# lucidrains/voicebox-pytorch

Measured on AMD Instinct MI355X. Metric: mel-frames/sec train-step (fwd+bwd+allreduce+clip+Adam), higher is better.
Workload: dtype f16/bf16 (fp16 forward operands, bf16 backward operands, fp32 accumulate/master); 1 GPU; VoiceBox dim 512 depth 12 heads 16 unconditional, 8x1024 frames per GPU, train; global_batch=8, seq_len=1024, parallelism=dp1

## Files before the change

### include/vbx.h

```cpp
#ifndef VBX_H
#define VBX_H
#include <stddef.h>
#include <stdint.h>

#ifdef __cplusplus
extern "C" {
#endif

#define VBX_VERSION 1

enum { VBX_OK = 0, VBX_EINVAL = -1, VBX_EUNSUPPORTED = -2, VBX_EWORKSPACE = -3 };

int vbx_version(void);
const char* vbx_last_error(void);
int vbx_check_device(int dev);

enum { VBX_GEMM_NT = 0, VBX_GEMM_NN = 1, VBX_GEMM_TN = 2 };

enum {
  VBX_EPI_BF16 = 0,
  VBX_EPI_F32 = 1,
  VBX_EPI_QKV = 2,
  VBX_EPI_GEGLU = 3,
  VBX_EPI_SPLITK = 4,
// ... 426 lines not shown

size_t vbx_model_wpack_bytes(const vbx_model* m);
size_t vbx_model_act_bytes(const vbx_model* m);
int vbx_model_pack_weights(const vbx_model* m, void* stream);
int vbx_model_adaln_factors(const vbx_model* m, const float** dada, const float** temb, long* w_off, void** dst_f16);
long vbx_model_sq_partials(const vbx_model* m, long* ranges );
int vbx_model_adam_segments(const vbx_model* m, long n_flat, vbx_adam_seg* out, int max_segs, long* total_blocks);
int vbx_model_forward(const vbx_model* m, const vbx_io* io, void* stream);
int vbx_model_adaln_table(const vbx_model* m, const float* temb, int n, float* ada, void* stream);
int vbx_model_backward_head(const vbx_model* m, const vbx_io* io, const float* gscale, void* stream);
int vbx_model_backward_layer(const vbx_model* m, const vbx_io* io, int layer, void* stream);
int vbx_model_backward_embed(const vbx_model* m, const vbx_io* io, void* stream);
int vbx_wgrad_overlap(int on);
int vbx_wgrad_overlap_forks(void);
int vbx_wgrad_overlap_delay(float side_us, float main_us);

void* vbx_model_debug_ptr(const vbx_model* m, const char* name, int layer);

int vbx_split3_f16(const float* src, long rows, int K, long ld, void* dst_f16, int Kp, void* stream);
int vbx_pack_weight3(const float* src, int src_rows, int src_cols, void* dst_f16, int dst_rows, int dst_cols, int rowmap, int F,
                     void* stream);
int vbx_qknorm_rope_f32(const float* raw, int B, int H, int Np, float qk_scale, const float* q_gamma, const float* k_gamma,
                        const float* rot_cos, const float* rot_sin, float* q32, float* k32, float* v32, void* q16, void* k16,
                        void* qb, void* kb, void* v_bf16, void* v16, float* q_rnorm, float* k_rnorm,
                        float q16_scale ,
                        void* stream);
int vbx_attn_fwd_f32(const float* q, const float* k, const float* v, const uint8_t* mask, float* out32, void* out16, void* out_bf16,
                     float* lse, int B, int H, int Np, float scale, void* stream);
int vbx_attn_fwd_f32_dropout(const float* q, const float* k, const float* v, const uint8_t* mask, float* out32, void* out16,
                             void* out_bf16, float* lse, int B, int H, int Np, float scale, const void* bits_rm, float p, void* stream);
// ... 22 lines not shown
```

### voicebox-pytorch_amd/csrc/runtime.hip

```cpp
#include "common.hpp"
#include "wgrad_overlap_plan.hpp"
#include <stdlib.h>
#include <algorithm>
#include <string.h>
#include <string>
#include <vector>

namespace {

inline size_t al256(size_t x) { return (x + 255) & ~(size_t)255; }

struct Carver {
  char* base;
  size_t off = 0;
  explicit Carver(void* b) : base((char*)b) {}
  template <class T>
  T* take(size_t n) {
    off = al256(off);
    T* p = base ? (T*)(base + off) : nullptr;
    off += n * sizeof(T);
    return p;
  }
};

// ... 295 lines not shown
  }
  ~ProfScope() {
    if (idx >= 0) (void)hipEventRecord(g_prof.recs[idx].e1, st);
  }
};

#define CK(x)                 \
  do {                        \
    int rc__ = (x);           \
    if (rc__ != 0) return rc__; \
  } while (0)

struct WgoSide {
  hipStream_t st = nullptr;
  hipEvent_t ev[wgrad_overlap::EV_N] = {};
};
int g_wgo_on = -1;
float g_wgo_delay[2] = {0.f, 0.f};
int g_wgo_forks = 0;
bool wgo_enabled() {
  if (g_wgo_on < 0) {
    const char* e = getenv("VBX_WGRAD_OVERLAP");
    g_wgo_on = e ? (atoi(e) != 0) : 1;
  }
  return g_wgo_on != 0;
}
WgoSide* wgo_side(bool create) {
  static WgoSide* sides[64] = {};
  int dev = 0;
  if (hipGetDevice(&dev) != hipSuccess || dev < 0 || dev >= 64) return nullptr;
  if (sides[dev] || !create) return sides[dev];
  WgoSide* s = new WgoSide;
  int least = 0, greatest = 0;
  bool ok = hipDeviceGetStreamPriorityRange(&least, &greatest) == hipSuccess &&
            hipStreamCreateWithPriority(&s->st, hipStreamNonBlocking, least) == hipSuccess;
  for (int i = 0; ok && i < wgrad_overlap::EV_N; i++) ok = hipEventCreateWithFlags(&s->ev[i], hipEventDisableTiming) == hipSuccess;
  if (!ok) {
    for (auto e : s->ev) if (e) (void)hipEventDestroy(e);
    if (s->st) (void)hipStreamDestroy(s->st);
    delete s;
    (void)hipGetLastError();
    return nullptr;
  }
  return sides[dev] = s;
}
bool capturing(hipStream_t st) {
  hipStreamCaptureStatus cs = hipStreamCaptureStatusNone;
  return hipStreamIsCapturing(st, &cs) != hipSuccess || cs != hipStreamCaptureStatusNone;
}
int wgo_sync(WgoSide* sd, hipStream_t main_st, wgrad_overlap::Point p, int l, int L) {
  if (!sd) return 0;
  const wgrad_overlap::Sync s = wgrad_overlap::sync_at(p, l, L);
  if (s.kind == wgrad_overlap::SYNC_NONE) return 0;
  hipStream_t st = s.stream == wgrad_overlap::MAIN ? main_st : sd->st;
  const hipError_t e = s.kind == wgrad_overlap::SYNC_RECORD ? hipEventRecord(sd->ev[s.ev], st) : hipStreamWaitEvent(st, sd->ev[s.ev], 0);
  VBX_REQUIRE(e == hipSuccess, "weight-gradient overlap: event %s failed (%s)", s.kind == wgrad_overlap::SYNC_RECORD ? "record" : "wait",
              hipGetErrorString(e));
  return 0;
}
struct WgoGuard {
  WgoSide* sd = nullptr;
  bool forked = false, ok = false;
  int done(int rc) { ok = rc == 0; return rc; }
  ~WgoGuard() {
    if (forked && !ok && sd) (void)hipStreamSynchronize(sd->st);
  }
};
bool defers(const vbx_model* m) { return m->defer_reduce && !m->gateloop && !m->unet && (m->plain_norm || m->adaln_factors); }
struct { const void* act = nullptr; int dxb = 0, dqkv = 0; } g_last_copy;

int check_model(const vbx_model* m) {
  VBX_REQUIRE(m && m->params && m->off && m->wpack && m->act && m->rot_cos && m->rot_sin, "vbx_model: null field");
  VBX_REQUIRE(m->D % 64 == 0 && m->D <= 2048, "vbx_model: dim must be a multiple of 64 and <= 2048 (got %d)", m->D);
  VBX_REQUIRE(m->H > 0 && m->H % 2 == 0, "vbx_model: heads must be even (dim_head is fixed at 64)");
  VBX_REQUIRE(m->Th % 8 == 0 && m->L > 0 && m->B > 0 && m->N > 0 && m->R >= 0 && m->F > 0, "vbx_model: bad dims");
  VBX_REQUIRE(m->ksize >= 1 && m->ksize <= 31 && (m->ksize & 1), "vbx_model: conv_pos_embed_kernel_size must be odd and <= 31 (got %d)", m->ksize);
  VBX_REQUIRE(m->E >= 0 && m->E % 8 == 0 && (m->E == 0 || (m->V1 > 0 && !m->stack_only)), "vbx_model: bad dim_cond_emb / table size");
  const long DT = (long)m->D * m->Th;
  for (int l = 0; l < m->L; l++) {
    const long* o = m->off + VBX_NG + (long)l * VBX_NL;
    if (m->plain_norm) continue;
    VBX_REQUIRE(o[VBX_L_B1W] == o[VBX_L_G1W] + DT && o[VBX_L_G2W] == o[VBX_L_B1W] + DT && o[VBX_L_B2W] == o[VBX_L_G2W] + DT,
                "vbx_model: adaLN weights of layer %d are not contiguous in (g1,b1,g2,b2) order", l);
// ... 146 lines not shown
  const float* P = m->params;
  const long* G = m->off;
  const bool tr = m->training != 0;

  if (m->precise) {
    std::vector<VbxPreciseLayer> pl(d.L);
    for (int l = 0; l < d.L; l++) {
      const ALayer& y = a.layer[l];
      pl[l] = VbxPreciseLayer{y.hn1, y.q16, y.k16, y.qb, y.kb, y.v, y.vh, y.oh, y.o, y.hn2, y.gh, y.g, tr ? y.h1 : nullptr,
                              y.qrn, y.krn, y.lse, w.layer[l].b1, y.hg, y.glp, y.gls, tr ? y.glh : nullptr, (unsigned*)y.dbr, (unsigned*)y.dbc};
    }
    VbxPreciseActs pa{a.four, a.pre, a.temb, a.ada, a.e, a.pred, a.per_b, a.xs.data(), pl.data(), a.embed_in, a.embed_inh, a.hf};
    return vbx_forward_precise(m, io, &pa, stream);
  }

  if (m->stack_only) {
    CK(vbx_stack_input(io->x, d.R ? P + G[VBX_P_REG] : nullptr, a.xs[0], d.B, d.N, d.R, d.D, stream));
    if (!m->plain_norm) CK(vbx_adaln_proj_fwd(io->cond, w.adah, w.bada, a.ada, d.B, d.Th, d.J, 4 * d.D, stream));
  } else {
  if (io->ada_table) {
    VBX_REQUIRE(!tr && io->ada_counter && io->ada_stride >= 1,
                "vbx_model_forward: ada_table is an inference-only input and needs ada_counter and ada_stride >= 1");
    CK(vbx_ada_select(a.ada, d.L, d.B, 4 * d.D, io->ada_table, io->ada_counter, io->ada_stride, io->ada_slot, stream));
  } else {
  CK(vbx_time_embed_fwd(io->times, P + G[VBX_P_SINW], P + G[VBX_P_T1W], P + G[VBX_P_T1B], a.four, a.pre, a.temb, d.B, d.D,
                        d.Th, stream));
  CK(vbx_adaln_proj_fwd(a.temb, w.adah, w.bada, a.ada, d.B, d.Th, d.J, 4 * d.D, stream));
  }
  if (d.Lc) {
    CK(vbx_proj_in_embed(io->x, io->cond, w.pinh, P + G[VBX_P_PINB], io->cond_mask, io->drop_mask, io->null_cond, a.embed_inh,
                         a.embed_in, a.xcb, d.B, d.N, d.Lc, d.D, d.E, stream));
    if (d.E) {
      VBX_REQUIRE(io->cond_ids && io->T > 0, "vbx_model_forward: a text-conditioned model needs cond_ids");
      CK(vbx_embed_text_cols(io->drop_mask, io->cond_ids, io->T, P + G[VBX_P_CEMB], d.E, io->null_id, a.embed_inh, a.embed_in, d.B,
                             d.N, d.D, d.Ke, stream));
    }
  } else if (d.E) {
    VBX_REQUIRE(io->cond_ids && io->T > 0, "vbx_model_forward: a text-conditioned model needs cond_ids");
    CK(vbx_pack_embed_input_text(io->x, io->cond, io->cond_mask, io->drop_mask, io->null_cond, io->cond_ids, io->T,
                                 P + G[VBX_P_CEMB], d.E, io->null_id, a.embed_inh, a.embed_in, d.B, d.N, d.Din, stream));
  } else {
    CK(vbx_pack_embed_input(io->x, io->cond, io->cond_mask, a.embed_inh, a.embed_in, d.B, d.N, d.Din, stream));
  }
  CK(gemm_nt(a.embed_inh, d.Ke, w.embh, d.Ke, (int)d.M0, d.D, d.Ke, VBX_EPI_F32, a.e, d.D, P + G[VBX_P_EMBB], nullptr,
             nullptr, nullptr, st));
  if (m->packed)
    CK(vbx_convpos_fwd_segs(a.e, P + G[VBX_P_CONVW], P + G[VBX_P_CONVB], d.R ? P + G[VBX_P_REG] : nullptr, io->seg_start, io->seg_klen,
                            io->tile_seg, a.xs[0], d.N, d.R, d.D, d.ks, stream));
  else
  CK(vbx_convpos_fwd(a.e, P + G[VBX_P_CONVW], P + G[VBX_P_CONVB], io->attn_mask, d.R ? P + G[VBX_P_REG] : nullptr, a.xs[0],
                     d.B, d.N, d.R, d.D, d.ks, stream));
  }

  for (int l = 0; l < d.L; l++) {
    const long* o = m->off + VBX_NG + (long)l * VBX_NL;
    const ALayer& y = a.layer[l];
    const float* ada_l = a.ada + (size_t)l * d.B * 4 * d.D;
    const int S = m->gateloop ? 3 : 2;
    float* x0 = layer_input(m, a, l);
    float* x_in = m->gateloop ? a.xs[S * l + 1] : x0;
    float* x_mid = a.xs[S * l + S - 1];
    float* x_out = a.xs[S * l + S];
    if (m->unet && l >= d.L / 2) {
      CK(vbx_unet_cat(a.xs[S * l], a.xs[S * (d.L - 1 - l)], m->skip_scale, a.cat16, nullptr, d.M, d.D, stream));
      CK(gemm_nt(a.cat16, 2 * d.D, w.layer[l].skwh, 2 * d.D, (int)d.M, d.D, 2 * d.D, VBX_EPI_F32, x0, d.D, P + o[VBX_L_SKB], nullptr,
                 nullptr, nullptr, st));
    }
    if (m->gateloop) {
// ... 39 lines not shown
    if (drop_on && m->ff_dropout > 0.f)
      CK(vbx_dropout_rows(y.gh, tr ? y.g : nullptr, d.M, d.Fp, d.Fp, io->drop_seed, 2u * l + 1u, m->ff_dropout, stream));
    { ProfScope ps("fwd ff_out", st);
      CK(gemm_nt(y.gh, d.Fp, w.layer[l].w2h, d.Fp, (int)d.M, d.D, d.Fp, VBX_EPI_F32, x_out, d.D, P + o[VBX_L_FF2B], x_mid, nullptr,
                 nullptr, st)); }
  }
  if (m->stack_only)
    return vbx_rmsnorm_fwd_f32(a.xs[(m->gateloop ? 3 : 2) * d.L], P + G[VBX_P_FNG], nullptr, 0, io->pred, d.B, d.Np, d.R, d.N, d.D,
                               stream);
  CK(vbx_rmsnorm_fwd(a.xs[(m->gateloop ? 3 : 2) * d.L], P + G[VBX_P_FNG], nullptr, 0, a.hf, a.hfh, d.B, d.Np, m->packed ? 0 : d.R, d.N, d.D,
                     stream));
  if (d.Dop != d.Do) {
    CK(gemm_nt(a.hfh, d.D, w.predh, d.D, (int)d.M0, d.Dop, d.D, VBX_EPI_F32, a.pred, d.Dop, nullptr, nullptr, nullptr, nullptr, st));
    if (io->pred) CK(vbx_copy_cols_f32(a.pred, d.Dop, io->pred, d.M0, d.Do, stream));
    if (io->target) CK(vbx_masked_mse_fwd_ld(a.pred, d.Dop, io->target, io->loss_mask, a.per_b, io->loss, d.B, d.N, d.Do, stream));
    return 0;
  }
  float* pred = io->pred ? io->pred : a.pred;
  CK(gemm_nt(a.hfh, d.D, w.predh, d.D, (int)d.M0, d.Do, d.D, VBX_EPI_F32, pred, d.Do, nullptr, nullptr, nullptr, nullptr, st));
  if (io->target) CK(vbx_masked_mse_fwd(pred, io->target, io->loss_mask, a.per_b, io->loss, d.B, d.N, d.Do, stream));
  return 0;
}

extern "C" int vbx_model_backward_head(const vbx_model* m, const vbx_io* io, const float* gscale, void* stream) {
  CK(check_model(m));
  VBX_REQUIRE(m->training && m->grads && io && io->target && (m->stack_only || io->loss_mask),
              "vbx_model_backward_head: needs a training forward");
  hipStream_t st = (hipStream_t)stream;
  const Dims d = dims_of(m);
  WPack w;
  carve_wpack(m, w);
  Acts a;
  carve_acts(m, a);
  const float* P = m->params;
  float* Gd = m->grads;
  const long* G = m->off;
  WgoGuard guard;
  guard.sd = capturing(st) ? nullptr : wgo_side(false);
  guard.forked = guard.sd != nullptr;
  CK(wgo_sync(guard.sd, st, wgrad_overlap::PT_HEAD_BEGIN, -1, d.L));
  u16* const dxb = defers(m) ? a.copy[wgrad_overlap::BUF_DXB][wgrad_overlap::dxb_read_copy(d.L - 1)] : a.dxb;
  g_last_copy.act = m->act; g_last_copy.dxb = (int)(dxb != a.dxb ? wgrad_overlap::dxb_read_copy(d.L - 1) : 0);
  if (m->stack_only) {
    CK(vbx_pack_weight(io->target, (int)d.M0, d.D, a.dhn, nullptr, (int)d.M0, d.D, 0, 0, stream));
  } else {
    const float* pred = io->pred ? io->pred : a.pred;
    if (d.Dop != d.Do)
      CK(vbx_masked_mse_bwd_ld(a.pred, d.Dop, io->target, io->loss_mask, a.per_b, gscale, a.dpb, d.B, d.N, d.Do, stream));
    else
      CK(vbx_masked_mse_bwd(pred, io->target, io->loss_mask, a.per_b, gscale, nullptr, a.dpb, d.B, d.N, d.Do, stream));
    CK(wgrad(a.dpb, d.Dop, a.hf, d.D, d.Dop, d.D, d.M0, a.slabs, Gd + G[VBX_P_PREDW], d.Do, d.D, 0, 0, st));
    CK(gemm_nn_bf16(a.dpb, d.Dop, w.pred, d.D, (int)d.M0, d.D, d.Dop, a.dhn, d.D, st));
  }
  if (hipMemsetAsync(a.dx, 0, (size_t)d.M * d.D * sizeof(float), st) != hipSuccess ||
      hipMemsetAsync(dxb, 0, (size_t)d.M * d.D * sizeof(u16), st) != hipSuccess) {
    vbx_set_error("vbx_model_backward_head: memset failed");
    return VBX_EINVAL;
  }
  CK(vbx_rmsnorm_bwd(a.xs[(m->gateloop ? 3 : 2) * d.L], P + G[VBX_P_FNG], 0, a.dhn, nullptr, a.dx, dxb, a.npart, nullptr, d.B, d.Np, d.R, d.N, d.D,
                     stream));
  CK(vbx_reduce_norm_partials(a.npart, a.tmp2d, 0, d.B, vbx_rmsnorm_bwd_chunks(d.N), d.D, 1, stream));
  CK(vbx_sum_rows_f32(a.tmp2d, 1, d.D, Gd + G[VBX_P_FNG], d.D, 0, stream));
  return guard.done(0);
}

struct SqLayout { long off[4], per_layer; };
static SqLayout sq_layout(const Dims& d) {
  SqLayout q;
  const long n[4] = {vbx_splitk_reduce_blocks(d.D, d.Fp), vbx_splitk_reduce_blocks(2 * d.Fp, d.D), vbx_splitk_reduce_blocks(d.D, d.I),
                     vbx_splitk_reduce_blocks(3 * d.I, d.D)};
  q.off[0] = 0;
  for (int i = 1; i < 4; i++) q.off[i] = q.off[i - 1] + n[i - 1];
  q.per_layer = q.off[3] + n[3];
  return q;
}
extern "C" long vbx_model_sq_partials(const vbx_model* m, long* ranges) {
  if (check_model(m) != 0) return 0;
// ... 139 lines not shown
  namespace wgo = wgrad_overlap;
  auto copy_of = [&](wgo::Buf b) { return pl.defer ? a.copy[b][wgo::write_copy(b, l)] : a.copy[b][0]; };
  u16* const dxb_in = pl.defer ? a.copy[wgo::BUF_DXB][wgo::dxb_read_copy(l)] : a.dxb;
  u16* const dxb_out = copy_of(wgo::BUF_DXB);
  u16* const dh1 = copy_of(wgo::BUF_DH1);
  u16* const dqkv = copy_of(wgo::BUF_DQKV);
  u16* dxb_attn = wgp ? copy_of(wgo::BUF_DXB2) : dxb_in;
  g_last_copy.act = m->act; g_last_copy.dxb = pl.defer ? wgo::write_copy(wgo::BUF_DXB, l) : 0; g_last_copy.dqkv = pl.defer ? wgo::write_copy(wgo::BUF_DQKV, l) : 0;
  const bool cap = capturing(st);
  const bool fork = pl.defer && wgp && wgo_enabled() && !g_prof.on && !cap;
  WgoGuard guard;
  guard.sd = cap ? nullptr : wgo_side(fork);
  VBX_REQUIRE(!fork || guard.sd, "vbx_model_backward_layer: could not create the weight-gradient side stream");
  if (fork && g_wgo_delay[1] > 0.f) CK(vbx_stream_delay(g_wgo_delay[1], stream));
  CK(wgo_sync(guard.sd, st, wgo::PT_LAYER_BEGIN, l, d.L));
  float* const slabs = fork ? a.slabs_side : a.slabs;
  const size_t sfl = a.slab_floats;
  const SqLayout sql = sq_layout(d);
  float* const sqb = m->sq_partials ? m->sq_partials + (long)l * sql.per_layer : nullptr;
  auto sq_at = [&](int i) { return sqb ? sqb + sql.off[i] : nullptr; };

  { ProfScope ps("dgrad ff_out", st); CK(gemm_nn_bf16(dxb_in, d.D, wl.w2, d.Fp, M, d.Fp, d.D, a.dg, d.Fp, st)); }
  CK(wgrad(dxb_in, d.D, y.g, d.Fp, d.D, d.Fp, d.M, slabs, Gd + o[VBX_L_FF2W], d.D, d.F, 0, 0, st, &wj, wgp, gs, sq_at(0)));
  if (drop_on && m->ff_dropout > 0.f)
    CK(vbx_dropout_rows(nullptr, a.dg, d.M, d.Fp, d.Fp, io->drop_seed, 2u * l + 1u, m->ff_dropout, stream));
  CK(vbx_geglu_bwd_colsum(y.h1, a.dg, dh1, M, d.Fp, csl, stream));
  { ProfScope ps("dgrad ff_in", st); CK(gemm_nn_bf16(dh1, 2 * d.Fp, wl.w1, d.D, M, d.D, 2 * d.Fp, a.dhn, d.D, st)); }
  CK(wgrad(dh1, 2 * d.Fp, y.hn2, d.D, 2 * d.Fp, d.D, d.M, slabs + sfl, Gd + o[VBX_L_FF1W], 2 * d.F, d.D, 1, d.F, st, &wj, wgp, gs, sq_at(1)));
  CK(vbx_rmsnorm_bwd(x_mid, g2, gstride, a.dhn, a.dx, a.dx, dxb_attn, npart, cpart, d.B, d.Np, 0, d.Np, d.D, stream));

// ... 20 lines not shown
    if (g_wgo_delay[0] > 0.f) CK(vbx_stream_delay(g_wgo_delay[0], side));
    if (wgg.n) CK(vbx_gemm_tn_splitk_grouped(wgg.d, wgg.n, side));
    CK(wgo_sync(guard.sd, st, wgo::PT_SIDE_GEMM_DONE, l, d.L));
    if (wj.n) CK(vbx_splitk_reduce_multi(&wj, side));
    CK(wgo_sync(guard.sd, st, wgo::PT_SIDE_REDUCE_DONE, l, d.L));
  } else {
    if (wgg.n) { ProfScope ps("wgrad (4 GEMMs)", st); CK(vbx_gemm_tn_splitk_grouped(wgg.d, wgg.n, stream)); }
    if (wj.n) { ProfScope ps("wgrad slab reduce", st); CK(vbx_splitk_reduce_multi(&wj, stream)); }
  }
  CK(vbx_rmsnorm_bwd(x_in, g1, gstride, a.dhn, a.dx, a.dx, dxb_out, npart2, nullptr, d.B, d.Np, 0, d.Np, d.D, stream));

  vbx_mr_jobs jb{};
  if (!pl.defer) {
    layer_reduce_jobs(m, d, a, pl, l, 0, jb);
    CK(vbx_multi_reduce(&jb, stream));
  } else if (l == 0) {
    ProfScope ps("partials reduce (all)", st);
    for (int ll = d.L - 1; ll >= 0; ll--) {
      layer_reduce_jobs(m, d, a, pl, ll, ll, jb);
      if (jb.n + 8 > VBX_MR_MAX || ll == 0) {
        CK(vbx_multi_reduce(&jb, stream));
        jb.n = 0;
      }
    }
  }

  if (m->gateloop) CK(backward_gateloop(m, d, w, a, l, stream));
  if (m->unet) CK(backward_unet(m, d, w, a, l, stream));
  if (m->plain_norm) return guard.done(0);
  if (pl.ada_all) {
    if (l == 0) {
      ProfScope ps("adaLN dtemb (all)", st);
      CK(vbx_adaln_dtemb_all(w.adah, a.dada, a.dtemb, a.ada_scratch, d.L, d.B, d.Th, 4 * d.D, stream));
    }
    return guard.done(0);
  }
  return guard.done(vbx_adaln_proj_bwd(m->stack_only ? io->cond : a.temb, w.adah + (size_t)l * 4 * d.D * d.Th, dada_l,
                            m->adaln_factors ? nullptr : Gd + o[VBX_L_G1W], Gd + o[VBX_L_G1B], a.dtemb,
                            a.ada_scratch, d.B, d.Th, 4 * d.D, l == d.L - 1 ? 0 : 1, stream));
}

extern "C" int vbx_model_backward_embed(const vbx_model* m, const vbx_io* io, void* stream) {
  CK(check_model(m));
  VBX_REQUIRE(m->training && m->grads && io && (m->stack_only ? io->dx != nullptr : io->times != nullptr),
              "vbx_model_backward_embed: needs a training forward");
  hipStream_t st = (hipStream_t)stream;
  const Dims d = dims_of(m);
  WPack w;
  carve_wpack(m, w);
  Acts a;
  carve_acts(m, a);
  const float* P = m->params;
  float* Gd = m->grads;
  const long* G = m->off;
  WgoGuard guard;
  guard.sd = capturing(st) ? nullptr : wgo_side(false);
  guard.forked = guard.sd != nullptr;
  if (m->stack_only) {
    CK(vbx_stack_input_bwd(a.dx, io->dx, d.R ? Gd + G[VBX_P_REG] : nullptr, d.B, d.N, d.R, d.D, stream));
    if (!m->plain_norm && io->dcond &&
        hipMemcpyAsync(io->dcond, a.dtemb, (size_t)d.B * d.Th * sizeof(float), hipMemcpyDeviceToDevice, st) != hipSuccess) {
      vbx_set_error("vbx_model_backward_embed: copy of d(cond) failed");
      return VBX_EINVAL;
    }
    return guard.done(wgo_sync(guard.sd, st, wgrad_overlap::PT_EMBED_END, -1, d.L));
  }
  CK(vbx_convpos_bwd(a.e, P + G[VBX_P_CONVW], P + G[VBX_P_CONVB], io->attn_mask, a.dx, a.dpre, a.de, a.deb, a.wpart,
                     d.R ? Gd + G[VBX_P_REG] : nullptr, d.B, d.N, d.R, d.D, d.ks, stream));
  CK(vbx_conv_wgrad_finalize(a.wpart, vbx_convpos_bwd_chunks(d.B, d.N), d.D, d.ks, Gd + G[VBX_P_CONVW], Gd + G[VBX_P_CONVB], stream));
  CK(wgrad(a.deb, d.D, a.embed_in, d.Ke, d.D, d.Ke, d.M0, a.slabs, Gd + G[VBX_P_EMBW], d.D, d.Ke, 0, 0, st));
  if (d.E) {
    WPack w;
    carve_wpack(m, w);
    CK(gemm_nn_bf16(a.deb, d.D, w.embb + d.Din, d.Ke, (int)d.M0, d.E, d.D, a.demb, d.E, st));
    if (hipMemsetAsync(Gd + G[VBX_P_CEMB], 0, (size_t)m->V1 * d.E * sizeof(float), st) != hipSuccess) {
      vbx_set_error("vbx_model_backward_embed: memset of the embedding gradient failed");
      return VBX_EINVAL;
    }
    CK(vbx_cond_emb_bwd(a.demb, d.E, io->cond_ids, io->T, io->drop_mask, io->null_id, Gd + G[VBX_P_CEMB], d.B, d.N, d.E, stream));
  }
  if (d.Lc) {
    WPack w;
    carve_wpack(m, w);
    CK(gemm_nn_bf16(a.deb, d.D, w.embb, d.Ke, (int)d.M0, d.D, d.D, a.dxc, d.D, st));
    CK(gemm_nn_bf16(a.deb, d.D, w.embb + d.D + d.E, d.Ke, (int)d.M0, d.D, d.D, a.dxc + (size_t)d.M0 * d.D, d.D, st));
    vbx_gemm_desc g{};
    g.mode = VBX_GEMM_TN; g.epilogue = VBX_EPI_SPLITK; g.M = d.D; g.N = d.Kp; g.K = (int)(2 * d.M0); g.lda = d.D; g.ldb = d.Kp;
    g.A = a.dxc; g.B = a.xcb; g.C = a.slabs; g.splits = wgrad_splits(d.D, d.Kp, 2 * d.M0);
    CK(vbx_gemm(&g, st));
    CK(vbx_proj_in_wgrad_reduce(a.slabs, g.splits, d.D, d.Lc, Gd + G[VBX_P_PINW], Gd + G[VBX_P_PINB], stream));
  }
  CK(vbx_colsum_f32(a.de, (int)d.M0, d.D, d.D, Gd + G[VBX_P_EMBB], a.cs_scratch, stream));
  CK(vbx_time_embed_bwd(io->times, P + G[VBX_P_SINW], P + G[VBX_P_T1W], a.four, a.pre, a.dtemb, Gd + G[VBX_P_SINW],
                        Gd + G[VBX_P_T1W], Gd + G[VBX_P_T1B], a.tscratch, d.B, d.D, d.Th, stream));
  return guard.done(wgo_sync(guard.sd, st, wgrad_overlap::PT_EMBED_END, -1, d.L));
}

extern "C" int vbx_model_adam_segments(const vbx_model* m, long n_flat, vbx_adam_seg* out, int max_segs, long* total_blocks) {
  CK(check_model(m));
  VBX_REQUIRE(n_flat > 0 && total_blocks, "vbx_model_adam_segments: bad args");
  const Dims d = dims_of(m);
  WPack w;
  carve_wpack(m, w);
  const long* G = m->off;
  std::vector<vbx_adam_seg> ps;
  auto add = [&](long off, long rows, long cols, void* b, void* h16, float* f32, int ld, int rowmap, int F) {
    vbx_adam_seg s{};
    s.off = off; s.count = rows * cols; s.dst_bf16 = b; s.dst_f16 = h16; s.dst_f32 = f32; s.cols = (int)cols; s.dst_ld = ld;
    s.rowmap = rowmap; s.F = F;
    ps.push_back(s);
// ... 55 lines not shown
}

extern "C" int vbx_wgrad_overlap(int on) {
  VBX_REQUIRE(on == 0 || on == 1, "vbx_wgrad_overlap: 0 in line, 1 on the side stream");
  g_wgo_on = on;
  return 0;
}
extern "C" int vbx_wgrad_overlap_forks(void) { return g_wgo_forks; }
extern "C" int vbx_wgrad_overlap_delay(float side_us, float main_us) {
  VBX_REQUIRE(side_us >= 0.f && side_us <= 2000.f && main_us >= 0.f && main_us <= 2000.f, "vbx_wgrad_overlap_delay: 0 .. 2000 us each");
  g_wgo_delay[0] = side_us;
  g_wgo_delay[1] = main_us;
  return 0;
}

extern "C" int vbx_prof_enable(int on) {
  for (auto& r : g_prof.recs) { (void)hipEventDestroy(r.e0); (void)hipEventDestroy(r.e1); }
  g_prof.recs.clear();
  g_prof.on = on != 0;
  return 0;
}
extern "C" int vbx_prof_collect(vbx_prof_entry* out, int max_entries) {
  VBX_REQUIRE(out && max_entries > 0, "vbx_prof_collect: bad args");
  g_prof.on = false;
  int n = 0;
  for (auto& r : g_prof.recs) {
    float ms = 0.f;
    if (hipEventSynchronize(r.e1) != hipSuccess || hipEventElapsedTime(&ms, r.e0, r.e1) != hipSuccess) continue;
    int k = 0;
    for (; k < n; k++)
// ... 39 lines not shown
```

Measured before the change: 1.005 million mel-frames/s.

## Move small independent step branches onto an auxiliary stream with event joins

Adds a second low-priority auxiliary stream and an event plan that moves small independent launches off the main stream. In backward these are the to_pred weight gradient, the final-norm gradient reduce, the grouped per-layer partial multi-reduces, the adaLN dtemb pass and the time-embedding backward. The forward head region is defined, but the plan's region_kept excludes it, so the time-embed and adaLN projection still run inline. The goal is to hide these latency-bound kernels behind main-stream GEMM work, at the cost of more event records and waits plus added cross-stream hazard complexity.

```diff
diff --git a/include/vbx.h b/include/vbx.h
--- a/include/vbx.h
+++ b/include/vbx.h
@@ -464,6 +464,9 @@
 int vbx_wgrad_overlap(int on);
 int vbx_wgrad_overlap_forks(void);
 int vbx_wgrad_overlap_delay(float side_us, float main_us);
+int vbx_step_branches(int on);
+int vbx_step_branches_forks(void);
+int vbx_step_branches_delay(float aux_us, float main_us);
 
 void* vbx_model_debug_ptr(const vbx_model* m, const char* name, int layer);
 
diff --git a/voicebox-pytorch_amd/csrc/runtime.hip b/voicebox-pytorch_amd/csrc/runtime.hip
--- a/voicebox-pytorch_amd/csrc/runtime.hip
+++ b/voicebox-pytorch_amd/csrc/runtime.hip
@@ -1,5 +1,6 @@
 #include "common.hpp"
 #include "wgrad_overlap_plan.hpp"
+#include "step_branches_plan.hpp"
 #include <stdlib.h>
 #include <algorithm>
 #include <string.h>
@@ -333,10 +334,15 @@
 struct WgoSide {
   hipStream_t st = nullptr;
   hipEvent_t ev[wgrad_overlap::EV_N] = {};
+  hipStream_t aux = nullptr;
+  hipEvent_t evb[step_branches::EV_N] = {};
 };
 int g_wgo_on = -1;
 float g_wgo_delay[2] = {0.f, 0.f};
 int g_wgo_forks = 0;
+int g_sb_on = 1;
+float g_sb_delay[2] = {0.f, 0.f};
+int g_sb_forks = 0;
 bool wgo_enabled() {
   if (g_wgo_on < 0) {
     const char* e = getenv("VBX_WGRAD_OVERLAP");
@@ -352,11 +358,15 @@
   WgoSide* s = new WgoSide;
   int least = 0, greatest = 0;
   bool ok = hipDeviceGetStreamPriorityRange(&least, &greatest) == hipSuccess &&
-            hipStreamCreateWithPriority(&s->st, hipStreamNonBlocking, least) == hipSuccess;
+            hipStreamCreateWithPriority(&s->st, hipStreamNonBlocking, least) == hipSuccess &&
+            hipStreamCreateWithPriority(&s->aux, hipStreamNonBlocking, least) == hipSuccess;
   for (int i = 0; ok && i < wgrad_overlap::EV_N; i++) ok = hipEventCreateWithFlags(&s->ev[i], hipEventDisableTiming) == hipSuccess;
+  for (int i = 0; ok && i < step_branches::EV_N; i++) ok = hipEventCreateWithFlags(&s->evb[i], hipEventDisableTiming) == hipSuccess;
   if (!ok) {
     for (auto e : s->ev) if (e) (void)hipEventDestroy(e);
+    for (auto e : s->evb) if (e) (void)hipEventDestroy(e);
     if (s->st) (void)hipStreamDestroy(s->st);
+    if (s->aux) (void)hipStreamDestroy(s->aux);
     delete s;
     (void)hipGetLastError();
     return nullptr;
@@ -377,15 +387,40 @@
               hipGetErrorString(e));
   return 0;
 }
+int sb_sync(WgoSide* sd, hipStream_t main_st, step_branches::Point p, int l, int L, int per_layer, bool on) {
+  if (!sd) return 0;
+  const step_branches::Sync s = step_branches::sync_at(p, l, L, per_layer, on);
+  if (s.kind == step_branches::SYNC_NONE) return 0;
+  hipStream_t st = s.stream == step_branches::MAIN ? main_st : sd->aux;
+  const hipError_t e = s.kind == step_branches::SYNC_RECORD ? hipEventRecord(sd->evb[s.ev], st) : hipStreamWaitEvent(st, sd->evb[s.ev], 0);
+  VBX_REQUIRE(e == hipSuccess, "step branches: event %s failed (%s)", s.kind == step_branches::SYNC_RECORD ? "record" : "wait",
+              hipGetErrorString(e));
+  return 0;
+}
 struct WgoGuard {
   WgoSide* sd = nullptr;
   bool forked = false, ok = false;
   int done(int rc) { ok = rc == 0; return rc; }
   ~WgoGuard() {
-    if (forked && !ok && sd) (void)hipStreamSynchronize(sd->st);
+    if (forked && !ok && sd) {
+      (void)hipStreamSynchronize(sd->st);
+      (void)hipStreamSynchronize(sd->aux);
+    }
   }
 };
 bool defers(const vbx_model* m) { return m->defer_reduce && !m->gateloop && !m->unet && (m->plain_norm || m->adaln_factors); }
+bool sb_backward(const vbx_model* m, bool cap) {
+  return g_sb_on && defers(m) && group_wgrad() && wgo_enabled() && !g_prof.on && !cap && !m->stack_only && !m->precise;
+}
+int sb_fork(WgoGuard& guard, hipStream_t main_st, step_branches::Point fork, step_branches::Point begin, int l, int L, int per_layer) {
+  CK(sb_sync(guard.sd, main_st, fork, l, L, per_layer, true));
+  guard.forked = true;
+  g_sb_forks++;
+  if (g_sb_delay[1] > 0.f) CK(vbx_stream_delay(g_sb_delay[1], main_st));
+  CK(sb_sync(guard.sd, main_st, begin, l, L, per_layer, true));
+  if (g_sb_delay[0] > 0.f) CK(vbx_stream_delay(g_sb_delay[0], guard.sd->aux));
+  return 0;
+}
 struct { const void* act = nullptr; int dxb = 0, dqkv = 0; } g_last_copy;
 
 int check_model(const vbx_model* m) {
@@ -562,6 +597,15 @@
     return vbx_forward_precise(m, io, &pa, stream);
   }
 
+  namespace sb = step_branches;
+  WgoGuard guard;
+  const bool branch = tr && sb::region_on(sb::REG_FWD_HEAD, g_sb_on != 0) && !m->stack_only && !m->gateloop && !m->unet && !io->ada_table &&
+                      group_wgrad() && wgo_enabled() && !g_prof.on && !capturing(st);
+  if (branch) {
+    guard.sd = wgo_side(true);
+    VBX_REQUIRE(guard.sd, "vbx_model_forward: could not create the side streams");
+  }
+
   if (m->stack_only) {
     CK(vbx_stack_input(io->x, d.R ? P + G[VBX_P_REG] : nullptr, a.xs[0], d.B, d.N, d.R, d.D, stream));
     if (!m->plain_norm) CK(vbx_adaln_proj_fwd(io->cond, w.adah, w.bada, a.ada, d.B, d.Th, d.J, 4 * d.D, stream));
@@ -571,9 +615,12 @@
                 "vbx_model_forward: ada_table is an inference-only input and needs ada_counter and ada_stride >= 1");
     CK(vbx_ada_select(a.ada, d.L, d.B, 4 * d.D, io->ada_table, io->ada_counter, io->ada_stride, io->ada_slot, stream));
   } else {
+  if (branch) CK(sb_fork(guard, st, sb::PT_FWD_BEGIN, sb::PT_FWD_AUX_BEGIN, -1, d.L, 0));
+  void* const ts = branch ? (void*)guard.sd->aux : stream;
   CK(vbx_time_embed_fwd(io->times, P + G[VBX_P_SINW], P + G[VBX_P_T1W], P + G[VBX_P_T1B], a.four, a.pre, a.temb, d.B, d.D,
-                        d.Th, stream));
-  CK(vbx_adaln_proj_fwd(a.temb, w.adah, w.bada, a.ada, d.B, d.Th, d.J, 4 * d.D, stream));
+                        d.Th, ts));
+  CK(vbx_adaln_proj_fwd(a.temb, w.adah, w.bada, a.ada, d.B, d.Th, d.J, 4 * d.D, ts));
+  CK(sb_sync(guard.sd, st, sb::PT_FWD_AUX_END, -1, d.L, 0, branch));
   }
   if (d.Lc) {
     CK(vbx_proj_in_embed(io->x, io->cond, w.pinh, P + G[VBX_P_PINB], io->cond_mask, io->drop_mask, io->null_cond, a.embed_inh,
@@ -600,6 +647,7 @@
                      d.B, d.N, d.R, d.D, d.ks, stream));
   }
 
+  CK(sb_sync(guard.sd, st, sb::PT_FWD_LAYER0, -1, d.L, 0, branch));
   for (int l = 0; l < d.L; l++) {
     const long* o = m->off + VBX_NG + (long)l * VBX_NL;
     const ALayer& y = a.layer[l];
@@ -669,12 +717,12 @@
     CK(gemm_nt(a.hfh, d.D, w.predh, d.D, (int)d.M0, d.Dop, d.D, VBX_EPI_F32, a.pred, d.Dop, nullptr, nullptr, nullptr, nullptr, st));
     if (io->pred) CK(vbx_copy_cols_f32(a.pred, d.Dop, io->pred, d.M0, d.Do, stream));
     if (io->target) CK(vbx_masked_mse_fwd_ld(a.pred, d.Dop, io->target, io->loss_mask, a.per_b, io->loss, d.B, d.N, d.Do, stream));
-    return 0;
+    return guard.done(0);
   }
   float* pred = io->pred ? io->pred : a.pred;
   CK(gemm_nt(a.hfh, d.D, w.predh, d.D, (int)d.M0, d.Do, d.D, VBX_EPI_F32, pred, d.Do, nullptr, nullptr, nullptr, nullptr, st));
   if (io->target) CK(vbx_masked_mse_fwd(pred, io->target, io->loss_mask, a.per_b, io->loss, d.B, d.N, d.Do, stream));
-  return 0;
+  return guard.done(0);
 }
 
 extern "C" int vbx_model_backward_head(const vbx_model* m, const vbx_io* io, const float* gscale, void* stream) {
@@ -690,10 +738,15 @@
   const float* P = m->params;
   float* Gd = m->grads;
   const long* G = m->off;
+  namespace sb = step_branches;
+  const bool cap = capturing(st);
+  const bool branch = sb::region_on(sb::REG_BWD_HEAD, sb_backward(m, cap));
   WgoGuard guard;
-  guard.sd = capturing(st) ? nullptr : wgo_side(false);
+  guard.sd = cap ? nullptr : wgo_side(branch);
+  VBX_REQUIRE(!branch || guard.sd, "vbx_model_backward_head: could not create the side streams");
   guard.forked = guard.sd != nullptr;
   CK(wgo_sync(guard.sd, st, wgrad_overlap::PT_HEAD_BEGIN, -1, d.L));
+  CK(sb_sync(guard.sd, st, sb::PT_HEAD_BEGIN, -1, d.L, 0, branch));
   u16* const dxb = defers(m) ? a.copy[wgrad_overlap::BUF_DXB][wgrad_overlap::dxb_read_copy(d.L - 1)] : a.dxb;
   g_last_copy.act = m->act; g_last_copy.dxb = (int)(dxb != a.dxb ? wgrad_overlap::dxb_read_copy(d.L - 1) : 0);
   if (m->stack_only) {
@@ -704,7 +757,7 @@
       CK(vbx_masked_mse_bwd_ld(a.pred, d.Dop, io->target, io->loss_mask, a.per_b, gscale, a.dpb, d.B, d.N, d.Do, stream));
     else
       CK(vbx_masked_mse_bwd(pred, io->target, io->loss_mask, a.per_b, gscale, nullptr, a.dpb, d.B, d.N, d.Do, stream));
-    CK(wgrad(a.dpb, d.Dop, a.hf, d.D, d.Dop, d.D, d.M0, a.slabs, Gd + G[VBX_P_PREDW], d.Do, d.D, 0, 0, st));
+    if (!branch) CK(wgrad(a.dpb, d.Dop, a.hf, d.D, d.Dop, d.D, d.M0, a.slabs, Gd + G[VBX_P_PREDW], d.Do, d.D, 0, 0, st));
     CK(gemm_nn_bf16(a.dpb, d.Dop, w.pred, d.D, (int)d.M0, d.D, d.Dop, a.dhn, d.D, st));
   }
   if (hipMemsetAsync(a.dx, 0, (size_t)d.M * d.D * sizeof(float), st) != hipSuccess ||
@@ -714,8 +767,16 @@
   }
   CK(vbx_rmsnorm_bwd(a.xs[(m->gateloop ? 3 : 2) * d.L], P + G[VBX_P_FNG], 0, a.dhn, nullptr, a.dx, dxb, a.npart, nullptr, d.B, d.Np, d.R, d.N, d.D,
                      stream));
-  CK(vbx_reduce_norm_partials(a.npart, a.tmp2d, 0, d.B, vbx_rmsnorm_bwd_chunks(d.N), d.D, 1, stream));
-  CK(vbx_sum_rows_f32(a.tmp2d, 1, d.D, Gd + G[VBX_P_FNG], d.D, 0, stream));
+  hipStream_t hs = st;
+  if (branch) {
+    CK(sb_fork(guard, st, sb::PT_HEAD_FORK, sb::PT_HEAD_AUX_BEGIN, -1, d.L, 0));
+    hs = guard.sd->aux;
+    CK(wgrad(a.dpb, d.Dop, a.hf, d.D, d.Dop, d.D, d.M0, a.slabs, Gd + G[VBX_P_PREDW], d.Do, d.D, 0, 0, hs));
+  }
+  CK(vbx_reduce_norm_partials(a.npart, a.tmp2d, 0, d.B, vbx_rmsnorm_bwd_chunks(d.N), d.D, 1, hs));
+  CK(vbx_sum_rows_f32(a.tmp2d, 1, d.D, Gd + G[VBX_P_FNG], d.D, 0, hs));
+  CK(sb_sync(guard.sd, st, sb::PT_HEAD_AUX_DONE, -1, d.L, 0, branch));
+  CK(sb_sync(guard.sd, st, sb::PT_HEAD_AUX_JOIN, -1, d.L, 0, branch));
   return guard.done(0);
 }
 
@@ -885,6 +946,9 @@
   VBX_REQUIRE(!fork || guard.sd, "vbx_model_backward_layer: could not create the weight-gradient side stream");
   if (fork && g_wgo_delay[1] > 0.f) CK(vbx_stream_delay(g_wgo_delay[1], stream));
   CK(wgo_sync(guard.sd, st, wgo::PT_LAYER_BEGIN, l, d.L));
+  namespace sb = step_branches;
+  const bool tail = fork && sb::region_on(sb::REG_BWD_TAIL, sb_backward(m, cap));
+  CK(sb_sync(guard.sd, st, sb::PT_LAYER_BEGIN, l, d.L, 0, tail));
   float* const slabs = fork ? a.slabs_side : a.slabs;
   const size_t sfl = a.slab_floats;
   const SqLayout sql = sq_layout(d);
@@ -935,6 +999,20 @@
   if (!pl.defer) {
     layer_reduce_jobs(m, d, a, pl, l, 0, jb);
     CK(vbx_multi_reduce(&jb, stream));
+  } else if (tail) {
+    layer_reduce_jobs(m, d, a, pl, l, l, jb);
+    const int per_layer = jb.n;
+    jb.n = 0;
+    const int first = sb::mr_group_first(l, d.L, per_layer);
+    if (first >= 0) {
+      static_assert(sb::kMrMax == VBX_MR_MAX, "step_branches_plan.hpp restates VBX_MR_MAX");
+      VBX_REQUIRE((first - l + 1) * per_layer <= VBX_MR_MAX, "vbx_model_backward_layer: the reduce plan overfills a launch");
+      CK(sb_fork(guard, st, sb::PT_MR_FORK, sb::PT_MR_AUX_BEGIN, l, d.L, per_layer));
+      for (int ll = first; ll >= l; ll--) layer_reduce_jobs(m, d, a, pl, ll, ll, jb);
+      CK(vbx_multi_reduce(&jb, guard.sd->aux));
+      if (l == 0 && pl.ada_all) CK(vbx_adaln_dtemb_all(w.adah, a.dada, a.dtemb, a.ada_scratch, d.L, d.B, d.Th, 4 * d.D, guard.sd->aux));
+      CK(sb_sync(guard.sd, st, sb::PT_MR_AUX_END, l, d.L, per_layer, true));
+    }
   } else if (l == 0) {
     ProfScope ps("partials reduce (all)", st);
     for (int ll = d.L - 1; ll >= 0; ll--) {
@@ -950,7 +1028,7 @@
   if (m->unet) CK(backward_unet(m, d, w, a, l, stream));
   if (m->plain_norm) return guard.done(0);
   if (pl.ada_all) {
-    if (l == 0) {
+    if (l == 0 && !tail) {
       ProfScope ps("adaLN dtemb (all)", st);
       CK(vbx_adaln_dtemb_all(w.adah, a.dada, a.dtemb, a.ada_scratch, d.L, d.B, d.Th, 4 * d.D, stream));
     }
@@ -974,9 +1052,16 @@
   const float* P = m->params;
   float* Gd = m->grads;
   const long* G = m->off;
+  namespace sb = step_branches;
+  const bool cap = capturing(st);
   WgoGuard guard;
-  guard.sd = capturing(st) ? nullptr : wgo_side(false);
+  guard.sd = cap ? nullptr : wgo_side(false);
   guard.forked = guard.sd != nullptr;
+  const bool tail = guard.sd && sb::region_on(sb::REG_BWD_TAIL, sb_backward(m, cap));
+  auto join = [&]() -> int {
+    CK(wgo_sync(guard.sd, st, wgrad_overlap::PT_EMBED_END, -1, d.L));
+    return sb_sync(guard.sd, st, sb::PT_EMBED_END, -1, d.L, 0, tail);
+  };
   if (m->stack_only) {
     CK(vbx_stack_input_bwd(a.dx, io->dx, d.R ? Gd + G[VBX_P_REG] : nullptr, d.B, d.N, d.R, d.D, stream));
     if (!m->plain_norm && io->dcond &&
@@ -984,7 +1069,18 @@
       vbx_set_error("vbx_model_backward_embed: copy of d(cond) failed");
       return VBX_EINVAL;
     }
-    return guard.done(wgo_sync(guard.sd, st, wgrad_overlap::PT_EMBED_END, -1, d.L));
+    return guard.done(join());
+  }
+  auto time_bwd = [&](void* s) {
+    return vbx_time_embed_bwd(io->times, P + G[VBX_P_SINW], P + G[VBX_P_T1W], a.four, a.pre, a.dtemb, Gd + G[VBX_P_SINW],
+                              Gd + G[VBX_P_T1W], Gd + G[VBX_P_T1B], a.tscratch, d.B, d.D, d.Th, s);
+  };
+  if (tail) {
+    g_sb_forks++;
+    if (g_sb_delay[0] > 0.f) CK(vbx_stream_delay(g_sb_delay[0], guard.sd->aux));
+    CK(time_bwd(guard.sd->aux));
+    CK(sb_sync(guard.sd, st, sb::PT_EMBED_AUX_END, -1, d.L, 0, true));
+    if (g_sb_delay[1] > 0.f) CK(vbx_stream_delay(g_sb_delay[1], stream));
   }
   CK(vbx_convpos_bwd(a.e, P + G[VBX_P_CONVW], P + G[VBX_P_CONVB], io->attn_mask, a.dx, a.dpre, a.de, a.deb, a.wpart,
                      d.R ? Gd + G[VBX_P_REG] : nullptr, d.B, d.N, d.R, d.D, d.ks, stream));
@@ -1012,9 +1108,8 @@
     CK(vbx_proj_in_wgrad_reduce(a.slabs, g.splits, d.D, d.Lc, Gd + G[VBX_P_PINW], Gd + G[VBX_P_PINB], stream));
   }
   CK(vbx_colsum_f32(a.de, (int)d.M0, d.D, d.D, Gd + G[VBX_P_EMBB], a.cs_scratch, stream));
-  CK(vbx_time_embed_bwd(io->times, P + G[VBX_P_SINW], P + G[VBX_P_T1W], a.four, a.pre, a.dtemb, Gd + G[VBX_P_SINW],
-                        Gd + G[VBX_P_T1W], Gd + G[VBX_P_T1B], a.tscratch, d.B, d.D, d.Th, stream));
-  return guard.done(wgo_sync(guard.sd, st, wgrad_overlap::PT_EMBED_END, -1, d.L));
+  if (!tail) CK(time_bwd(stream));
+  return guard.done(join());
 }
 
 extern "C" int vbx_model_adam_segments(const vbx_model* m, long n_flat, vbx_adam_seg* out, int max_segs, long* total_blocks) {
@@ -1100,6 +1195,19 @@
   return 0;
 }
 
+extern "C" int vbx_step_branches(int on) {
+  VBX_REQUIRE(on == 0 || on == 1, "vbx_step_branches: 0 in line, 1 on the AUX stream");
+  g_sb_on = on;
+  return 0;
+}
+extern "C" int vbx_step_branches_forks(void) { return g_sb_forks; }
+extern "C" int vbx_step_branches_delay(float aux_us, float main_us) {
+  VBX_REQUIRE(aux_us >= 0.f && aux_us <= 2000.f && main_us >= 0.f && main_us <= 2000.f, "vbx_step_branches_delay: 0 .. 2000 us each");
+  g_sb_delay[0] = aux_us;
+  g_sb_delay[1] = main_us;
+  return 0;
+}
+
 extern "C" int vbx_prof_enable(int on) {
   for (auto& r : g_prof.recs) { (void)hipEventDestroy(r.e0); (void)hipEventDestroy(r.e1); }
   g_prof.recs.clear();
diff --git a/voicebox-pytorch_amd/csrc/step_branches_plan.hpp b/voicebox-pytorch_amd/csrc/step_branches_plan.hpp
--- /dev/null
+++ b/voicebox-pytorch_amd/csrc/step_branches_plan.hpp
@@ -0,0 +1,282 @@
+#pragma once
+#include <string.h>
+
+#include "wgrad_overlap_plan.hpp"
+
+namespace step_branches {
+namespace wgo = wgrad_overlap;
+
+enum Stream { MAIN = wgo::MAIN, SIDE = wgo::SIDE, AUX, STREAM_N };
+
+enum Region { REG_FWD_HEAD, REG_BWD_HEAD, REG_BWD_TAIL, REG_N };
+constexpr bool region_kept(Region r) { return r != REG_FWD_HEAD; }
+
+enum Launch { LA_TIME_EMBED_FWD, LA_ADALN_PROJ_FWD, LA_TO_PRED_WGRAD, LA_FNORM_REDUCE, LA_MULTI_REDUCE, LA_ADALN_DTEMB, LA_TIME_EMBED_BWD };
+constexpr Region region_of(Launch la) {
+  return la <= LA_ADALN_PROJ_FWD ? REG_FWD_HEAD : (la <= LA_FNORM_REDUCE ? REG_BWD_HEAD : REG_BWD_TAIL);
+}
+constexpr bool region_on(Region r, bool on) { return on && region_kept(r); }
+constexpr Stream stream_of(Launch la, bool on) { return region_on(region_of(la), on) ? AUX : MAIN; }
+
+constexpr int kMrMax = 48, kMrRoom = 8;
+constexpr int mr_group_first(int l, int L, int per_layer) {
+  int n = 0, first = L - 1;
+  for (int ll = L - 1; ll >= 0; ll--) {
+    n += per_layer;
+    if (n + kMrRoom > kMrMax || ll == 0) {
+      if (ll == l) return first;
+      n = 0;
+      first = ll - 1;
+    }
+  }
+  return -1;
+}
+
+enum Event { EV_FWD_FORK, EV_FWD_JOIN, EV_HEAD_FORK, EV_HEAD_DONE, EV_MR_FORK, EV_AUX_JOIN, EV_N };
+enum Point {
+  PT_FWD_BEGIN,
+  PT_FWD_AUX_BEGIN,
+  PT_FWD_AUX_END,
+  PT_FWD_LAYER0,
+  PT_HEAD_BEGIN,
+  PT_HEAD_FORK,
+  PT_HEAD_AUX_BEGIN,
+  PT_HEAD_AUX_DONE,
+  PT_HEAD_AUX_JOIN,
+  PT_LAYER_BEGIN,
+  PT_MR_FORK,
+  PT_MR_AUX_BEGIN,
+  PT_MR_AUX_END,
+  PT_EMBED_AUX_END,
+  PT_EMBED_END,
+  PT_N
+};
+using wgo::SYNC_NONE;
+using wgo::SYNC_RECORD;
+using wgo::SYNC_WAIT;
+using wgo::SyncKind;
+struct Sync {
+  SyncKind kind;
+  Stream stream;
+  Event ev;
+};
+constexpr Sync kNoSync{SYNC_NONE, MAIN, EV_N};
+constexpr Sync sync_at(Point p, int l, int L, int per_layer, bool on) {
+  switch (p) {
+    case PT_FWD_BEGIN: return region_on(REG_FWD_HEAD, on) ? Sync{SYNC_RECORD, MAIN, EV_FWD_FORK} : kNoSync;
+    case PT_FWD_AUX_BEGIN: return region_on(REG_FWD_HEAD, on) ? Sync{SYNC_WAIT, AUX, EV_FWD_FORK} : kNoSync;
+    case PT_FWD_AUX_END: return region_on(REG_FWD_HEAD, on) ? Sync{SYNC_RECORD, AUX, EV_FWD_JOIN} : kNoSync;
+    case PT_FWD_LAYER0: return region_on(REG_FWD_HEAD, on) ? Sync{SYNC_WAIT, MAIN, EV_FWD_JOIN} : kNoSync;
+    case PT_HEAD_BEGIN: return {SYNC_WAIT, MAIN, EV_AUX_JOIN};
+    case PT_HEAD_FORK: return region_on(REG_BWD_HEAD, on) ? Sync{SYNC_RECORD, MAIN, EV_HEAD_FORK} : kNoSync;
+    case PT_HEAD_AUX_BEGIN: return region_on(REG_BWD_HEAD, on) ? Sync{SYNC_WAIT, AUX, EV_HEAD_FORK} : kNoSync;
+    case PT_HEAD_AUX_DONE: return region_on(REG_BWD_HEAD, on) ? Sync{SYNC_RECORD, AUX, EV_HEAD_DONE} : kNoSync;
+    case PT_HEAD_AUX_JOIN: return region_on(REG_BWD_HEAD, on) ? Sync{SYNC_RECORD, AUX, EV_AUX_JOIN} : kNoSync;
+    case PT_LAYER_BEGIN: return l == 0 ? Sync{SYNC_WAIT, MAIN, EV_HEAD_DONE} : kNoSync;
+    case PT_MR_FORK:
+      return region_on(REG_BWD_TAIL, on) && mr_group_first(l, L, per_layer) >= 0 ? Sync{SYNC_RECORD, MAIN, EV_MR_FORK} : kNoSync;
+    case PT_MR_AUX_BEGIN:
+      return region_on(REG_BWD_TAIL, on) && mr_group_first(l, L, per_layer) >= 0 ? Sync{SYNC_WAIT, AUX, EV_MR_FORK} : kNoSync;
+    case PT_MR_AUX_END:
+      return region_on(REG_BWD_TAIL, on) && mr_group_first(l, L, per_layer) >= 0 ? Sync{SYNC_RECORD, AUX, EV_AUX_JOIN} : kNoSync;
+    case PT_EMBED_AUX_END: return region_on(REG_BWD_TAIL, on) ? Sync{SYNC_RECORD, AUX, EV_AUX_JOIN} : kNoSync;
+    case PT_EMBED_END: return {SYNC_WAIT, MAIN, EV_AUX_JOIN};
+    case PT_N: break;
+  }
+  return kNoSync;
+}
+constexpr int forks_per_step(int L, int per_layer) {
+  int n = (region_kept(REG_FWD_HEAD) ? 1 : 0) + (region_kept(REG_BWD_HEAD) ? 1 : 0) + (region_kept(REG_BWD_TAIL) ? 1 : 0);
+  for (int l = 0; l < L && region_kept(REG_BWD_TAIL); l++) n += mr_group_first(l, L, per_layer) >= 0 ? 1 : 0;
+  return n;
+}
+
+enum ResKind {
+  RES_TEMB = 16,
+  RES_ADA,
+  RES_EMBED_IN,
+  RES_E,
+  RES_XS0,
+  RES_DPB,
+  RES_DHN,
+  RES_DX,
+  RES_NPART,
+  RES_NPART2,
+  RES_CPART,
+  RES_GPART,
+  RES_CS_LAYERS,
+  RES_DADA,
+  RES_DTEMB,
+  RES_ADA_SCRATCH,
+  RES_TMP2D,
+  RES_TSCRATCH,
+  RES_CS_SCRATCH,
+  RES_DE,
+  RES_WPART,
+  RES_GRAD_SMALL,
+  RES_GRAD_FNORM,
+  RES_GRAD_TIME,
+  RES_GRAD_CONV,
+  RES_GRAD_EMBED_B,
+};
+struct Res {
+  int kind, a, b;
+};
+constexpr int kMaxReads = 72, kMaxWrites = 32;
+struct Op {
+  enum Type { LAUNCH, SYNC } type;
+  int stream;
+  const char* name;
+  int layer;
+  bool own;
+  int point;
+  SyncKind kind;
+  int ev;
+  Res reads[kMaxReads], writes[kMaxWrites];
+  int nr, nw;
+};
+
+struct Ctx {
+  int L, per_layer;
+  bool on;
+};
+
+template <class F>
+inline void emit_sync(Point p, int l, const Ctx& c, F&& f) {
+  const Sync s = sync_at(p, l, c.L, c.per_layer, c.on);
+  if (s.kind == SYNC_NONE) return;
+  Op o{};
+  o.type = Op::SYNC; o.stream = s.stream; o.name = s.kind == SYNC_WAIT ? "wait" : "record"; o.layer = l; o.own = true; o.point = p;
+  o.kind = s.kind; o.ev = s.ev;
+  f(o);
+}
+inline Op launch(int st, const char* name, int l, std::initializer_list<Res> reads, std::initializer_list<Res> writes) {
+  Op o{};
+  o.type = Op::LAUNCH; o.stream = st; o.name = name; o.layer = l;
+  for (const Res& r : reads) o.reads[o.nr++] = r;
+  for (const Res& w : writes) o.writes[o.nw++] = w;
+  return o;
+}
+inline Op convert(const wgo::Op& w) {
+  Op o{};
+  o.type = w.type == wgo::Op::SYNC ? Op::SYNC : Op::LAUNCH; o.stream = w.stream; o.name = w.name; o.layer = w.layer; o.own = false;
+  o.point = w.point; o.kind = w.sync.kind; o.ev = w.sync.ev;
+  for (int i = 0; i < w.nr; i++) o.reads[o.nr++] = Res{(int)w.reads[i].kind, w.reads[i].a, w.reads[i].b};
+  for (int i = 0; i < w.nw; i++) o.writes[o.nw++] = Res{(int)w.writes[i].kind, w.writes[i].a, w.writes[i].b};
+  return o;
+}
+constexpr Res kActs{wgo::RES_FWD_ACTS, 0, 0};
+
+template <class F>
+inline void emit_forward_head(const Ctx& c, F&& f) {
+  emit_sync(PT_FWD_BEGIN, -1, c, f);
+  emit_sync(PT_FWD_AUX_BEGIN, -1, c, f);
+  f(launch(stream_of(LA_TIME_EMBED_FWD, c.on), "time_embed_fwd", -1, {}, {{RES_TEMB, 0, 0}}));
+  f(launch(stream_of(LA_ADALN_PROJ_FWD, c.on), "adaln_proj_fwd", -1, {{RES_TEMB, 0, 0}}, {{RES_ADA, 0, 0}}));
+  emit_sync(PT_FWD_AUX_END, -1, c, f);
+  f(launch(MAIN, "pack_embed_input", -1, {}, {{RES_EMBED_IN, 0, 0}}));
+  f(launch(MAIN, "to_embed GEMM", -1, {{RES_EMBED_IN, 0, 0}}, {{RES_E, 0, 0}}));
+  f(launch(MAIN, "convpos_fwd", -1, {{RES_E, 0, 0}}, {{RES_XS0, 0, 0}}));
+  emit_sync(PT_FWD_LAYER0, -1, c, f);
+  f(launch(MAIN, "forward layers, to_pred, loss", -1, {{RES_XS0, 0, 0}, {RES_ADA, 0, 0}}, {kActs}));
+}
+
+template <class F>
+inline void emit_head(const Ctx& c, F&& f) {
+  const int L = c.L;
+  const bool br = region_on(REG_BWD_HEAD, c.on);
+  const Res dxb{wgo::RES_BUF, wgo::BUF_DXB, wgo::dxb_read_copy(L - 1)};
+  const Op wgrad = launch(stream_of(LA_TO_PRED_WGRAD, c.on), "to_pred wgrad + reduce", -1, {{RES_DPB, 0, 0}, kActs},
+                          {{wgo::RES_SLABS_MAIN, 0, 0}, {wgo::RES_GRAD_HEAD, 0, 0}});
+  wgo::emit_sync(wgo::PT_HEAD_BEGIN, -1, L, [&](const wgo::Op& w) { f(convert(w)); });
+  emit_sync(PT_HEAD_BEGIN, -1, c, f);
+  f(launch(MAIN, "masked_mse_bwd", -1, {kActs}, {{RES_DPB, 0, 0}}));
+  if (!br) f(wgrad);
+  f(launch(MAIN, "dgrad to_pred", -1, {{RES_DPB, 0, 0}}, {{RES_DHN, 0, 0}}));
+  f(launch(MAIN, "memset dx, dxb", -1, {}, {{RES_DX, 0, 0}, dxb}));
+  f(launch(MAIN, "final norm backward", -1, {kActs, {RES_DHN, 0, 0}}, {{RES_DX, 0, 0}, dxb, {RES_NPART, 0, 0}}));
+  emit_sync(PT_HEAD_FORK, -1, c, f);
+  emit_sync(PT_HEAD_AUX_BEGIN, -1, c, f);
+  if (br) f(wgrad);
+  f(launch(stream_of(LA_FNORM_REDUCE, c.on), "reduce_norm_partials", -1, {{RES_NPART, 0, 0}}, {{RES_TMP2D, 0, 0}}));
+  f(launch(stream_of(LA_FNORM_REDUCE, c.on), "sum_rows", -1, {{RES_TMP2D, 0, 0}}, {{RES_GRAD_FNORM, 0, 0}}));
+  emit_sync(PT_HEAD_AUX_DONE, -1, c, f);
+  emit_sync(PT_HEAD_AUX_JOIN, -1, c, f);
+}
+
+inline Op multi_reduce(int st, int first, int last) {
+  Op o = launch(st, "multi_reduce", last, {}, {});
+  for (int ll = first; ll >= last; ll--) {
+    for (int k : {(int)RES_NPART, (int)RES_NPART2, (int)RES_CPART, (int)RES_GPART, (int)RES_CS_LAYERS}) o.reads[o.nr++] = Res{k, ll, 0};
+    o.writes[o.nw++] = Res{RES_DADA, ll, 0};
+    o.writes[o.nw++] = Res{RES_GRAD_SMALL, ll, 0};
+  }
+  return o;
+}
+inline Op adaln_dtemb_all(int st, int L) {
+  Op o = launch(st, "adaln_dtemb_all", 0, {}, {{RES_DTEMB, 0, 0}, {RES_ADA_SCRATCH, 0, 0}});
+  for (int ll = L - 1; ll >= 0; ll--) o.reads[o.nr++] = Res{RES_DADA, ll, 0};
+  return o;
+}
+
+template <class F>
+inline void emit_layer(int l, const Ctx& c, F&& f) {
+  const int L = c.L;
+  emit_sync(PT_LAYER_BEGIN, l, c, f);
+  wgo::emit_layer(l, L, [&](const wgo::Op& w) {
+    Op o = convert(w);
+    if (o.type == Op::LAUNCH) {
+      if (!strcmp(o.name, "GEGLU backward")) o.writes[o.nw++] = Res{RES_CS_LAYERS, l, 0};
+      if (!strcmp(o.name, "norm backward (ff)")) {
+        o.reads[o.nr++] = Res{RES_ADA, 0, 0}; o.reads[o.nr++] = Res{RES_DX, 0, 0};
+        o.writes[o.nw++] = Res{RES_DX, 0, 0}; o.writes[o.nw++] = Res{RES_NPART, l, 0}; o.writes[o.nw++] = Res{RES_CPART, l, 0};
+      }
+      if (!strcmp(o.name, "attention backward")) o.writes[o.nw++] = Res{RES_GPART, l, 0};
+      if (!strcmp(o.name, "norm backward (attn)")) {
+        o.reads[o.nr++] = Res{RES_ADA, 0, 0}; o.reads[o.nr++] = Res{RES_DX, 0, 0};
+        o.writes[o.nw++] = Res{RES_DX, 0, 0}; o.writes[o.nw++] = Res{RES_NPART2, l, 0};
+      }
+    }
+    f(o);
+  });
+  if (region_on(REG_BWD_TAIL, c.on)) {
+    const int first = mr_group_first(l, L, c.per_layer);
+    if (first < 0) return;
+    emit_sync(PT_MR_FORK, l, c, f);
+    emit_sync(PT_MR_AUX_BEGIN, l, c, f);
+    f(multi_reduce(AUX, first, l));
+    if (l == 0) f(adaln_dtemb_all(AUX, L));
+    emit_sync(PT_MR_AUX_END, l, c, f);
+  } else if (l == 0) {
+    for (int ll = L - 1; ll >= 0; ll--) {
+      const int first = mr_group_first(ll, L, c.per_layer);
+      if (first >= 0) f(multi_reduce(MAIN, first, ll));
+    }
+    f(adaln_dtemb_all(MAIN, L));
+  }
+}
+
+template <class F>
+inline void emit_embed(const Ctx& c, F&& f) {
+  const bool br = region_on(REG_BWD_TAIL, c.on);
+  const Op tbwd = launch(stream_of(LA_TIME_EMBED_BWD, c.on), "time_embed_bwd", -1, {{RES_DTEMB, 0, 0}, {RES_TEMB, 0, 0}},
+                         {{RES_GRAD_TIME, 0, 0}, {RES_TSCRATCH, 0, 0}});
+  if (br) f(tbwd);
+  emit_sync(PT_EMBED_AUX_END, -1, c, f);
+  f(launch(MAIN, "convpos_bwd", -1, {{RES_DX, 0, 0}, {RES_E, 0, 0}}, {{RES_DE, 0, 0}, {RES_WPART, 0, 0}, {RES_GRAD_CONV, 1, 0}}));
+  f(launch(MAIN, "conv_wgrad_finalize", -1, {{RES_WPART, 0, 0}}, {{RES_GRAD_CONV, 0, 0}}));
+  f(launch(MAIN, "to_embed wgrad + reduce", -1, {{RES_DE, 0, 0}, {RES_EMBED_IN, 0, 0}}, {{wgo::RES_SLABS_MAIN, 0, 0}, {wgo::RES_GRAD_EMBED, 0, 0}}));
+  f(launch(MAIN, "colsum", -1, {{RES_DE, 0, 0}}, {{RES_CS_SCRATCH, 0, 0}, {RES_GRAD_EMBED_B, 0, 0}}));
+  if (!br) f(tbwd);
+  wgo::emit_sync(wgo::PT_EMBED_END, -1, c.L, [&](const wgo::Op& w) { f(convert(w)); });
+  emit_sync(PT_EMBED_END, -1, c, f);
+}
+
+template <class F>
+inline void emit_backward(const Ctx& c, F&& f) {
+  emit_head(c, f);
+  for (int l = c.L - 1; l >= 0; l--) emit_layer(l, c, f);
+  emit_embed(c, f);
+}
+
+}
```

After: 1.013 million mel-frames/s (median of 6 runs). About the same (+0.9%).
